# duxfrederic/lightcurver

Hardware: AMD Instinct MI355X
Metric: cutouts/sec (PSF-fit + joint forward-model iter), 32x32 & 64x64 stamps (higher is better)
Workload: dtype f32

## Files before the change

### include/lcmi.h

```cpp
#ifndef LCMI_H
#define LCMI_H

#include <stdint.h>

#ifdef __cplusplus
extern "C" {
#endif

#define LC_OK 0
#define LC_ERR_INVALID (-1)
#define LC_ERR_DEVICE (-2)
#define LC_ERR_UNSUPPORTED (-3)
#define LC_ERR_NONFINITE (-4)

typedef struct lc_ctx lc_ctx;
typedef struct lc_psf_batch lc_psf_batch;
typedef struct lc_joint lc_joint;

int lc_version(void);
int lc_ctx_create(int device, lc_ctx **out);
void lc_ctx_destroy(lc_ctx *ctx);
const char *lc_last_error(const lc_ctx *ctx);
int lc_ctx_synchronize(lc_ctx *ctx);
int lc_ctx_stream(lc_ctx *ctx, void **hip_stream, int *device);
// ... 37 lines not shown
                      int32_t *status , float *kernel_ms );

typedef struct {
  float n_sigma;
  int32_t clip;
} lc_stack_cfg;
int lc_align_stack_supported(int n);
int lc_align_stack(lc_ctx *ctx, int C, int E, int n, const float *cubes ,
                   const float *noisemap ,
                   const double *shift_yx , const double *angle_deg , const lc_stack_cfg *cfg,
                   float *aligned , float *stack ,
                   float *median , int32_t *n_rejected ,
                   float *kernel_ms );

typedef struct {
  float init_learning_rate;
  int32_t schedule_learning_rate;
  float decay_rate;
  int32_t transition_steps;
  float b1, b2, eps, eps_root;
} lc_adabelief_cfg;
void lc_adabelief_defaults(lc_adabelief_cfg *cfg);

int lc_psf_supported(int n, int ss);
int lc_psf_batch_create(lc_ctx *ctx, int F, int S_max, int n, int ss, const float *data,
                        const float *weight, lc_psf_batch **out);
void lc_psf_batch_destroy(lc_psf_batch *b);
int lc_psf_batch_set_moffat(lc_psf_batch *b, const float *moffat);
int lc_psf_batch_get_moffat(lc_psf_batch *b, float *moffat);
int lc_psf_batch_set_stars(lc_psf_batch *b, const float *stars);
int lc_psf_batch_get_stars(lc_psf_batch *b, float *stars);
int lc_psf_batch_set_grid(lc_psf_batch *b, const float *grid);
int lc_psf_batch_get_grid(lc_psf_batch *b, float *grid);
int lc_psf_batch_set_regularization(lc_psf_batch *b, const float *W, float lam_scales, float lam_hf);
int lc_psf_batch_propagate_noise(lc_psf_batch *b);
int lc_psf_batch_get_weights(lc_psf_batch *b, float *W);
int lc_psf_batch_eval(lc_psf_batch *b, float *loss, float *chi2, float *grad_moffat,
                      float *grad_stars, float *grad_grid, float *model);
int lc_psf_batch_fit_moffat(lc_psf_batch *b, int n_iter, float *final_loss );
int lc_psf_batch_run_adabelief(lc_psf_batch *b, int n_iter, const lc_adabelief_cfg *cfg);
int lc_psf_batch_iterations_done(lc_psf_batch *b);
int lc_psf_batch_split_fallbacks(lc_psf_batch *b, int *count);
int lc_psf_batch_get_loss_history(lc_psf_batch *b, float *history, int stride);
int lc_psf_batch_get_results(lc_psf_batch *b, float *narrow_psf, float *full_psf, float *residuals,
                             float *chi2);

int lc_psf_batch_set_moffat_q(lc_psf_batch *b, const float *q );
int lc_psf_batch_set_distortion(lc_psf_batch *frames, int S_stars, const float *coeffs ,
                                const float *xy );
int lc_psf_distortion_forward(lc_psf_batch *frames, lc_psf_batch *stars);
int lc_psf_distortion_backward(lc_psf_batch *frames, lc_psf_batch *stars);
int lc_psf_batch_get_ext_grad(lc_psf_batch *b, float *grad );
int lc_psf_batch_step_adabelief(lc_psf_batch *b, const lc_adabelief_cfg *cfg, int use_ext_grad, int export_grad);
int lc_psf_distortion_run(lc_psf_batch *frames, lc_psf_batch *stars, int n_iter, const lc_adabelief_cfg *cfg);
int lc_batched_lbfgs(int nb, int D, double *x, const double *lo, const double *hi, int maxiter,
                     int (*eval)(void *user, const double *X, double *F, double *G), void *user,
                     double *f_final , int *evaluations );

int lc_apply_distortion(lc_ctx *ctx, int N, int K, const float *narrow_psf, const float *coeffs,
                        const float *xy, float *out);

enum { LC_P_A = 0, LC_P_CX = 1, LC_P_CY = 2, LC_P_DX = 3, LC_P_DY = 4, LC_P_ALPHA = 5, LC_P_H = 6,
       LC_P_MEAN = 7, LC_P_COUNT = 8 };

typedef struct {
  float lam_scales, lam_hf;
// ... 72 lines not shown
```

### lightcurver_amd/_lib.py

```python
import ctypes as C
import os

import numpy as np

_HERE = os.path.dirname(os.path.abspath(__file__))
LIB_PATH = os.path.join(_HERE, 'liblcmi.so')

P_A, P_CX, P_CY, P_DX, P_DY, P_ALPHA, P_H, P_MEAN, P_COUNT = range(9)
PARAM_INDEX = {'a': P_A, 'c_x': P_CX, 'c_y': P_CY, 'dx': P_DX, 'dy': P_DY, 'alpha': P_ALPHA,
               'h': P_H, 'mean': P_MEAN}

fp = C.POINTER(C.c_float)
dp = C.POINTER(C.c_double)
ip = C.POINTER(C.c_int32)
vp = C.c_void_p
LBFGS_EVAL = C.CFUNCTYPE(C.c_int, C.c_void_p, dp, dp, dp)
ALLREDUCE_FN = C.CFUNCTYPE(C.c_int, C.c_void_p, C.c_void_p, C.c_int, C.c_void_p)
IPC_HANDLE_BYTES = 64
RCCL_ID_BYTES = 128


class AdabeliefCfg(C.Structure):
    _fields_ = [('init_learning_rate', C.c_float), ('schedule_learning_rate', C.c_int32),
                ('decay_rate', C.c_float), ('transition_steps', C.c_int32),
# ... 27 lines not shown
SIGNATURES = {
    'lc_version': (C.c_int, []),
    'lc_ctx_create': (C.c_int, [C.c_int, C.POINTER(vp)]),
    'lc_ctx_destroy': (None, [vp]),
    'lc_last_error': (C.c_char_p, [vp]),
    'lc_copy_bandwidth': (C.c_int, [vp, C.c_int64, C.c_int, C.POINTER(C.c_float)]),
    'lc_ctx_marker': (C.c_int, [vp, C.c_int]),
    'lc_prepare_stamps': (C.c_int, [vp, C.c_int, C.c_int, fp, fp, fp, fp, fp, C.POINTER(C.c_uint8), C.c_float, C.c_float,
                                    C.c_int, fp, fp, fp, C.POINTER(C.c_int32), C.POINTER(C.c_float)]),
    'lc_cosmics_supported': (C.c_int, [C.c_int]),
    'lc_detect_cosmics': (C.c_int, [vp, C.c_int, C.c_int, fp, fp, C.POINTER(C.c_uint8), C.POINTER(CosmicsCfg),
                                    C.POINTER(C.c_uint8), fp, ip, C.POINTER(C.c_float)]),
    'lc_segment_supported': (C.c_int, [C.c_int]),
    'lc_segment_stamps': (C.c_int, [vp, C.c_int, C.c_int, fp, fp, C.POINTER(SegmentCfg), C.POINTER(C.c_uint8), ip, ip, fp,
                                    ip, C.POINTER(C.c_float)]),
    'lc_align_stack_supported': (C.c_int, [C.c_int]),
    'lc_align_stack': (C.c_int, [vp, C.c_int, C.c_int, C.c_int, fp, fp, dp, dp, C.POINTER(StackCfg), fp, fp, fp, ip,
                                 C.POINTER(C.c_float)]),
    'lc_ctx_stream': (C.c_int, [vp, C.POINTER(C.c_void_p), C.POINTER(C.c_int)]),
    'lc_ctx_synchronize': (C.c_int, [vp]),
    'lc_timer_start': (C.c_int, [vp]),
    'lc_timer_stop': (C.c_int, [vp, fp]),
    'lc_device_info': (C.c_int, [vp, C.c_char_p, C.c_int, C.POINTER(C.c_int), C.POINTER(C.c_int64)]),
    'lc_adabelief_defaults': (None, [C.POINTER(AdabeliefCfg)]),
    'lc_psf_supported': (C.c_int, [C.c_int, C.c_int]),
    'lc_psf_batch_create': (C.c_int, [vp, C.c_int, C.c_int, C.c_int, C.c_int, fp, fp, C.POINTER(vp)]),
    'lc_psf_batch_destroy': (None, [vp]),
    'lc_psf_batch_set_moffat': (C.c_int, [vp, fp]),
    'lc_psf_batch_get_moffat': (C.c_int, [vp, fp]),
    'lc_psf_batch_set_stars': (C.c_int, [vp, fp]),
    'lc_psf_batch_get_stars': (C.c_int, [vp, fp]),
    'lc_psf_batch_set_grid': (C.c_int, [vp, fp]),
    'lc_psf_batch_get_grid': (C.c_int, [vp, fp]),
    'lc_psf_batch_set_regularization': (C.c_int, [vp, fp, C.c_float, C.c_float]),
    'lc_psf_batch_propagate_noise': (C.c_int, [vp]),
    'lc_psf_batch_get_weights': (C.c_int, [vp, fp]),
    'lc_psf_batch_eval': (C.c_int, [vp, fp, fp, fp, fp, fp, fp]),
    'lc_psf_batch_fit_moffat': (C.c_int, [vp, C.c_int, fp]),
    'lc_psf_batch_run_adabelief': (C.c_int, [vp, C.c_int, C.POINTER(AdabeliefCfg)]),
    'lc_psf_batch_iterations_done': (C.c_int, [vp]),
    'lc_psf_batch_split_fallbacks': (C.c_int, [vp, C.POINTER(C.c_int)]),
    'lc_psf_batch_get_loss_history': (C.c_int, [vp, fp, C.c_int]),
    'lc_psf_batch_get_results': (C.c_int, [vp, fp, fp, fp, fp]),
    'lc_psf_batch_set_moffat_q': (C.c_int, [vp, fp]),
    'lc_psf_batch_set_distortion': (C.c_int, [vp, C.c_int, fp, fp]),
    'lc_psf_distortion_forward': (C.c_int, [vp, vp]),
    'lc_psf_distortion_backward': (C.c_int, [vp, vp]),
    'lc_psf_batch_get_ext_grad': (C.c_int, [vp, fp]),
    'lc_psf_batch_step_adabelief': (C.c_int, [vp, C.POINTER(AdabeliefCfg), C.c_int, C.c_int]),
    'lc_psf_distortion_run': (C.c_int, [vp, vp, C.c_int, C.POINTER(AdabeliefCfg)]),
    'lc_batched_lbfgs': (C.c_int, [C.c_int, C.c_int, dp, dp, dp, C.c_int, LBFGS_EVAL, vp, dp, C.POINTER(C.c_int)]),
    'lc_apply_distortion': (C.c_int, [vp, C.c_int, C.c_int, fp, fp, fp, fp]),
    'lc_joint_supported': (C.c_int, [C.c_int, C.c_int]),
    'lc_joint_groups_background_supported': (C.c_int, [C.c_int, C.c_int]),
    'lc_joint_set_debug_global': (C.c_int, [C.c_int]),
    'lc_joint_create': (C.c_int, [vp, C.c_int, C.c_int, C.c_int, C.c_int, fp, fp, fp, C.POINTER(vp)]),
    'lc_joint_create_groups': (C.c_int, [vp, C.c_int, ip, C.c_int, C.c_int, C.c_int, fp, fp, fp, C.POINTER(vp)]),
    'lc_joint_create_groups_background': (C.c_int, [vp, C.c_int, ip, C.c_int, C.c_int, C.c_int, fp, fp, fp, C.POINTER(vp)]),
    'lc_joint_get_group_loss_history': (C.c_int, [vp, fp, C.c_int]),
    'lc_joint_destroy': (None, [vp]),
    'lc_joint_set_param': (C.c_int, [vp, C.c_int, fp, C.c_int]),
    'lc_joint_get_param': (C.c_int, [vp, C.c_int, fp, C.c_int]),
    'lc_joint_set_flux_reference': (C.c_int, [vp, fp, C.c_int]),
    'lc_joint_get_flux_reference': (C.c_int, [vp, fp, C.c_int]),
    'lc_joint_set_free': (C.c_int, [vp, ip]),
    'lc_joint_set_loss': (C.c_int, [vp, C.POINTER(JointLossCfg), fp]),
# ... 153 lines not shown
```

### lightcurver_amd/csrc/psf_batch.hip

```cpp
#include <cmath>
#include <cstring>

#include "lbfgs_host.h"
#include <thread>

#include "noise_host.h"
#include "starlet_norms.h"
#include <cstdlib>

#include "psf_kernels.h"
#include "psf_noise.h"
#include "psf_distort.h"
#include "psf_lbfgs.h"

using namespace lc;

struct lc_psf_batch {
  lc_ctx *ctx = nullptr;
  int F = 0, S = 0, n = 0, ss = 0, N = 0, J = 0;
  float *data = nullptr, *wgt = nullptr, *W = nullptr, *norms = nullptr, *Tm = nullptr;
  float *B = nullptr, *mB = nullptr, *sB = nullptr;
  float *stars = nullptr, *stars_m = nullptr, *stars_s = nullptr, *moffat = nullptr;
  float *hist = nullptr, *qscratch = nullptr;
  float *sched = nullptr;
// ... 536 lines not shown
}
int lc_psf_batch_get_moffat(lc_psf_batch *b, float *moffat) {
  if (!b || !moffat) return LC_ERR_INVALID;
  LC_ENTER(b->ctx);
  return d2h(b, moffat, b->moffat, (size_t)b->F * 4 * sizeof(float));
}
int lc_psf_batch_set_stars(lc_psf_batch *b, const float *stars) {
  if (!b || !stars) return LC_ERR_INVALID;
  LC_ENTER(b->ctx);
  return h2d(b, b->stars, stars, (size_t)b->F * b->S * 4 * sizeof(float));
}
int lc_psf_batch_get_stars(lc_psf_batch *b, float *stars) {
  if (!b || !stars) return LC_ERR_INVALID;
  LC_ENTER(b->ctx);
  return d2h(b, stars, b->stars, (size_t)b->F * b->S * 4 * sizeof(float));
}
int lc_psf_batch_set_grid(lc_psf_batch *b, const float *grid) {
  if (!b) return LC_ERR_INVALID;
  LC_ENTER(b->ctx);
  const size_t bytes = (size_t)b->F * b->N * b->N * sizeof(float);
  if (grid) return h2d(b, b->B, grid, bytes);
  LC_HIP(b->ctx, hipMemsetAsync(b->B, 0, bytes, b->ctx->stream));
  LC_HIP(b->ctx, hipMemsetAsync(b->mB, 0, bytes, b->ctx->stream));
  LC_HIP(b->ctx, hipMemsetAsync(b->sB, 0, bytes, b->ctx->stream));
  LC_HIP(b->ctx, hipMemsetAsync(b->stars_m, 0, (size_t)b->F * b->S * 4 * sizeof(float), b->ctx->stream));
  LC_HIP(b->ctx, hipMemsetAsync(b->stars_s, 0, (size_t)b->F * b->S * 4 * sizeof(float), b->ctx->stream));
  b->iters_done = 0;
  return LC_OK;
}
int lc_psf_batch_get_grid(lc_psf_batch *b, float *grid) {
  if (!b || !grid) return LC_ERR_INVALID;
  LC_ENTER(b->ctx);
  return d2h(b, grid, b->B, (size_t)b->F * b->N * b->N * sizeof(float));
}
int lc_psf_batch_set_regularization(lc_psf_batch *b, const float *W, float lam_scales, float lam_hf) {
  if (!b) return LC_ERR_INVALID;
  LC_ENTER(b->ctx);
  b->lam_sc = lam_scales;
  b->lam_hf = lam_hf;
  if (W) {
    int rc = h2d(b, b->W, W, (size_t)b->F * b->J * b->N * b->N * sizeof(float));
    if (rc) return rc;
    b->have_W = true;
  }
  return LC_OK;
}
namespace {
typedef void (*noise_fn)(int, int, const float *, const float *, const float *, float *);
noise_fn find_noise_kernel(int N, int ss) {
  if (N == 16 && ss == 1) return psf_noise_accumulate_kernel<16, 1>;
  if (N == 32 && ss == 2) return psf_noise_accumulate_kernel<32, 2>;
  if (N == 48 && ss == 2) return psf_noise_accumulate_kernel<48, 2>;
  if (N == 64 && ss == 2) return psf_noise_accumulate_kernel<64, 2>;
  if (N == 128 && ss == 2) return psf_noise_accumulate_kernel<128, 2>;
  return nullptr;
}
}

int lc_psf_batch_propagate_noise(lc_psf_batch *b) {
  if (!b) return LC_ERR_INVALID;
  LC_ENTER(b->ctx);
  const int F = b->F, S = b->S, N = b->N, n = b->n, ss = b->ss, J = b->J;
  const size_t NN = (size_t)N * N, nn = (size_t)n * n;
  if (!std::getenv("LCMI_NOISE_HOST")) {
    noise_fn fn = find_noise_kernel(N, ss);
    if (!fn) LC_FAIL(b->ctx, LC_ERR_UNSUPPORTED, "no noise-propagation kernel for this stamp size");
// ... 314 lines not shown
```

### lightcurver_amd/csrc/psf_kernels.h

```cpp
#pragma once
#include <utility>

#include "lc_common.h"
#include "starlet_device.h"

#ifndef LC_XPOLL_SLEEP
#define LC_XPOLL_SLEEP 2
#endif
namespace lc {
constexpr int kXFlagStride = 16;

#ifdef LC_STAMPS
__device__ long long g_stamps[128];
#define LC_STAMP(k)                                                      \
  do {                                                                   \
    if ((blockIdx.x == 0 || blockIdx.x == 8) && threadIdx.x == 0 && it == A.n_iter - 1)  \
      g_stamps[(k) + (blockIdx.x == 8 ? 64 : 0)] = clock64();            \
  } while (0)
#else
#define LC_STAMP(k) do {} while (0)
#endif


struct PsfArgs {
  int F, S, n_iter, t0, hist_stride, mode;
  const float *data, *wgt;
  const float *W;
  const float *norms;
  const float *Tm;
  float *B, *mB, *sB;
  float *stars, *stars_m, *stars_s;
  float *hist;
  float *qscratch;
  float *out_loss, *out_chi2, *out_gstars, *out_ggrid, *out_gT, *out_model;
  float lam_sc, lam_hf;
  lc_adabelief_cfg ab;
  float *xch;
  int *xflags, *xabort;
  int launch_seq, heal, force_abort_it;
  const float *bkB, *bkmB, *bksB, *bkstars, *bkstars_m, *bkstars_s;
// ... 27 lines not shown
               : "memory");
}
__device__ __forceinline__ void load_sc1_x4(const float *p, lc_v4f &a) {
  asm volatile("global_load_dwordx4 %0, %1, off sc1\n\ts_waitcnt vmcnt(0)" : "=&v"(a) : "v"(p) : "memory");
}
__device__ __forceinline__ float load_sc1_f(const float *p) {
  float v;
  asm volatile("global_load_dword %0, %1, off sc1\n\ts_waitcnt vmcnt(0)" : "=&v"(v) : "v"(p) : "memory");
  return v;
}


template <int N_, int SS_, int PX_, int SG_, bool WC_ = false, int JB_ = 8>
struct PsfCfg {
  static constexpr int N = N_, SS = SS_, PX = PX_, SG = SG_;
  static constexpr bool WC = WC_;
  static constexpr int n = N / SS;
  static constexpr int NTHR = N * N / PX;
  static constexpr int NW = (NTHR + kWave - 1) / kWave;
  static constexpr int NT = ntaps(SS);
  static constexpr int J = ilog2(N);
  static constexpr int LR = 8;
  static constexpr int LC = (JB_ * (N_ / SS_) / 4 >= 64) ? 4 : 2;
  static constexpr int LA = LC;
  static constexpr int TS = N + 1;
  static constexpr int RS = n + 1;
  static constexpr int OFF_T = 0;
  static constexpr int SZ_T = WC_ ? N * (N + 2 * (N / 4 + 10) + 1) : N * TS;
  static constexpr int OFF_R = OFF_T + SZ_T;
  static constexpr int SZ_R2 = SG * n * TS;
  static constexpr int VS = WC_ ? n + 3 : RS, VO = WC_ ? 1 : 0;
  static constexpr int SZ_V = SG * N * VS;
  static constexpr int JB = JB_;
  static constexpr int AP = N / 4 + 10;
  static constexpr int TSA = N + 2 * AP + 1;
  static constexpr int APR = AP / SS + 2;
  static constexpr int JBP = JB + 1;
  static constexpr int WSZ = JB * TSA + (n + 2 * APR) * JBP;
  static constexpr int SZ_VR = (SZ_V > StarletLds<N>::FLOATS) ? SZ_V : StarletLds<N>::FLOATS;
  static constexpr int OFF_WSC = OFF_R + SZ_VR;
  static constexpr int SZ_R = WC ? (SZ_VR + NW * WSZ) : ((2 * SZ_R2 > SZ_V) ? 2 * SZ_R2 : SZ_V);
  static constexpr int OFF_RES = OFF_R + SZ_R;
  static constexpr int SZ_RES = WC ? 0 : SG * n * n;
  static constexpr int OFF_TAPS = OFF_RES + SZ_RES;
  static constexpr int NTP = NT + 3;
  static constexpr int SZ_TAPS = (16 * 4 * NTP + 1) / 2 * 2 + 16 * 2 * NT * 2;
  static constexpr int OFF_TAPP = OFF_TAPS + (16 * 4 * NTP + 1) / 2 * 2;
  static constexpr int OFF_RED = OFF_TAPS + SZ_TAPS;
  static constexpr int IPS = n * n / LC;
  static constexpr int IPS_PAD = (IPS + kWave - 1) / kWave * kWave;
  static constexpr int SLOTS = IPS_PAD / kWave;
  static constexpr int SZ_REDX = 16 * NW;
  static constexpr int SZ_RED = (WC ? 16 * (n / JB) * 5 : SG * SLOTS * 5) + SZ_REDX + NW + 8;
  static constexpr int OFF_REDX = OFF_RED + (WC ? 16 * (n / JB) * 5 : SG * SLOTS * 5);
  static constexpr int OFF_REDW = OFF_REDX + SZ_REDX;
  static constexpr int OFF_STAR = OFF_RED + SZ_RED;
  static constexpr int MAXS = 16;
  static constexpr int SZ_STAR = MAXS * 20 + 16;
  static constexpr int LDS_FLOATS = OFF_STAR + SZ_STAR;
  static_assert(WC || StarletLds<N>::FLOATS <= SZ_T + SZ_R + SZ_RES, "starlet ping-pong buffers must fit over T + R + RES");
  static_assert(PX % SS == 0 && N % PX == 0 && n % LR == 0 && n % LC == 0 && n % LA == 0 && n % JB == 0, "tiling");
  static_assert(LDS_FLOATS * 4 <= 163840, "LDS");
  static_assert(OFF_TAPP % 2 == 0, "tap pairs are read as 64-bit words");
  static_assert(NTHR <= 1024 && NTHR % kWave == 0, "threads");
  static_assert(!WC_ || PX_ <= 8, "the WC layout keeps the pixel state in registers");
};


template <int SS, int NT>
__device__ inline void tap_entry(float delta, int k, float &tap, float &dtap, int &bq) {
  const int o = (int)nearbyintf(delta);
  const int base = o - kRg - (SS - 1);
  int q = base / SS;
  if (q * SS > base) --q;
  bq = q;
  const int m = q * SS + k;
  const float inv_s2 = 1.0f / (kSigmaG * kSigmaG);
  const float nrm = 0.3989422804014327f / kSigmaG;
  float a = 0.f, d = 0.f;
#pragma unroll
  for (int dv = 0; dv < SS; ++dv) {
    const int t = m + dv;
    if (t >= o - kRg && t <= o + kRg) {
      const float x = (float)t - delta;
      const float p = nrm * expf(-0.5f * x * x * inv_s2);
      a += p;
      d += p * x * inv_s2;
    }
  }
  tap = a;
  dtap = d;
}

template <class C, bool SPLIT = false>
__global__ __launch_bounds__(C::NTHR) void psf_fit_kernel(PsfArgs A) {
  constexpr int N = C::N, SS = C::SS, PX = C::PX, SG = C::SG, n = C::n, NT = C::NT, J = C::J;
  constexpr int NTHR = C::NTHR, TS = C::TS, RS = C::RS, LR = C::LR, LC = C::LC, LA = C::LA;
  extern __shared__ __align__(16) float lds[];
  float *T = lds + C::OFF_T;
  float *R2t = lds + C::OFF_R;
  float *R2xt = R2t + C::SZ_R2;
  float *V = lds + C::OFF_R;
  float *RES = lds + C::OFF_RES;
  float *TAPS = lds + C::OFF_TAPS + 1;
  constexpr int NTP = C::NTP;
  lc_v2f *TAPP = (lc_v2f *)(lds + C::OFF_TAPP);
  float *REDX = lds + C::OFF_REDX;
  float *RED = lds + C::OFF_RED;
  float *REDW = lds + C::OFF_REDW;
  float *SCAL = REDW + C::NW;
  float *SP = lds + C::OFF_STAR;
  float *SGR = SP + C::MAXS * 4;
  float *SM = SGR + C::MAXS * 5;
  float *SV = SM + C::MAXS * 4;
  int *BQ = (int *)(SV + C::MAXS * 4);

  int f = blockIdx.x, role = 0;
  if constexpr (SPLIT) {
    f = ((int)blockIdx.x >> 4) * 8 + ((int)blockIdx.x & 7);
    role = ((int)blockIdx.x >> 3) & 1;
    if (f >= A.F) return;
  }
  const bool conv_role = !SPLIT || role == 0, starlet_role = !SPLIT || role == 1;
  const int my_xcc = SPLIT ? (int)(__builtin_amdgcn_s_getreg(20 | (3 << 11)) & 15u) : 0;
  int same_xcd = 0;
  const int tid0 = threadIdx.x;
// ... 122 lines not shown
    float tpix[PX];
    if (conv_role) {
    if (C::WC && STATE_REGS) {
#pragma unroll
      for (int p = 0; p < PX; ++p) {
        tpix[p] = Bp[p] + Tp[p];
        T[pu * C::TSA + C::AP + pv + p] = tpix[p];
      }
    } else if (STATE_REGS) {
#pragma unroll
      for (int p = 0; p < PX; ++p) T[pu * TS + pv + p] = Bp[p] + Tp[p];
    } else {
      const float4 *bp = (const float4 *)(Bg + gpix);
      const float4 *tp = (const float4 *)(A.Tm + gpix);
#pragma unroll
      for (int q = 0; q < PX / 4; ++q) {
        const float4 b = bp[q], t = tp[q];
        T[pu * TS + pv + 4 * q + 0] = b.x + t.x;
        T[pu * TS + pv + 4 * q + 1] = b.y + t.y;
        T[pu * TS + pv + 4 * q + 2] = b.z + t.z;
        T[pu * TS + pv + 4 * q + 3] = b.w + t.w;
      }
    }
    if (tid < S * 5) SGR[tid] = 0.f;

    for (int g0 = 0; g0 < S; g0 += SG) {
      __syncthreads();
      LC_STAMP(1 + 5 * (g0 / SG));
      if constexpr (C::WC) {
        constexpr int JB = C::JB, NBLK = n / JB;
        float *wsc = lds + C::OFF_WSC + wid * C::WSZ;
        constexpr int TSA = C::TSA, AP = C::AP, APR = C::APR;
        float *R2w = wsc + AP, *RESw = wsc + JB * TSA + APR * C::JBP;
        int kdone = 0;
        for (int task = wid; task < SG * NBLK; task += C::NW, ++kdone) {
          progress_prio(kdone);
          const int sl = task / NBLK, blk = task % NBLK, s = g0 + sl;
          if (s >= S) continue;
          const int jd0 = blk * JB;
          const float *tx = TAPS + (s * 4 + 0) * NTP, *ty = tx + 2 * NTP, *dty = tx + 3 * NTP;
          const int bqx = BQ[s * 2 + 0], bqy = BQ[s * 2 + 1];
          const float amp = SP[s * 4 + 0], sky = SP[s * 4 + 3];
          constexpr int NI3 = (JB * (n / LC) + 63) / 64;
          float dpre[NI3][LC], wpre[NI3][LC];
#pragma unroll
          for (int i3 = 0; i3 < NI3; ++i3) {
            const int item = lane + 64 * i3;
            const bool ok = item < JB * (n / LC);
            const int jl = item % JB, a0 = (item / JB) * LC;
#pragma unroll
            for (int j = 0; j < LC; ++j) {
              const size_t pix = ok ? ((size_t)s * n * n + (size_t)(a0 + j) * n + jd0 + jl) : 0;
              const float dv = dataf[pix], wv = wgtf[pix];
              dpre[i3][j] = ok ? dv : 0.f;
              wpre[i3][j] = ok ? wv : 0.f;
            }
          }
          LC_STAMP(10);
          {
            const int ws = SS * (jd0 - bqx) - (NT - 1);
            if constexpr (SS == 2) {
              constexpr int NP = (NT + 1) / 2, WL2 = (JB - 1) + NP;
              lc_v2f tr2[NP];
#pragma unroll
              for (int h = 0; h < NP; ++h) tr2[h] = (lc_v2f){tx[NT - 1 - 2 * h], tx[NT - 2 - 2 * h]};
              for (int u = lane; u < N; u += 64) {
                lc_v2f win2[WL2];
                const float *trow = T + u * TSA + AP + ws;
#pragma unroll
                for (int i = 0; i < WL2; ++i) win2[i] = (lc_v2f){trow[2 * i], trow[2 * i + 1]};
                lc_v2f acc[JB];
#pragma unroll
                for (int j = 0; j < JB; ++j) acc[j] = (lc_v2f){0.f, 0.f};
#pragma unroll
                for (int h = 0; h < NP; ++h) {
#pragma unroll
                  for (int j = 0; j < JB; ++j) acc[j] = pk_fma(tr2[h], win2[j + h], acc[j]);
                }
#pragma unroll
                for (int j = 0; j < JB; ++j) R2w[j * TSA + u] = acc[j].x + acc[j].y;
              }
            } else {
              constexpr int WL = SS * (JB - 1) + NT;
              float tk[NT];
#pragma unroll
              for (int k = 0; k < NT; ++k) tk[k] = tx[k];
              for (int u = lane; u < N; u += 64) {
                float win[WL];
                const float *trow = T + u * TSA + AP + ws;
#pragma unroll
                for (int i = 0; i < WL; ++i) win[i] = trow[i];
#pragma unroll
                for (int j = 0; j < JB; ++j) {
                  float acc = 0.f;
#pragma unroll
                  for (int k = 0; k < NT; ++k) acc = fmaf(tk[k], win[SS * j - k + NT - 1], acc);
                  R2w[j * TSA + u] = acc;
                }
              }
            }
          }
          wave_lds_sync();
          LC_STAMP(11);
          float chi = 0.f, ga = 0.f, gy = 0.f, gs = 0.f;
          {
            constexpr int WL = SS * (LC - 1) + NT;
            lc_v2f tyd[NT];
#pragma unroll
            for (int k = 0; k < NT; ++k) tyd[k] = TAPP[(s * 2 + 1) * NT + k];
#pragma unroll
// ... 14 lines not shown
                for (int k = 0; k < NT; ++k) {
#pragma unroll
                  for (int j = 0; j < LC; ++j) fvys[j] = pk_fma(tyd[k], pk_bcast(win[SS * j - k + NT - 1]), fvys[j]);
                  if constexpr (LC == 4) asm volatile("" : "+v"(fvys[0]), "+v"(fvys[1]), "+v"(fvys[2]), "+v"(fvys[3]));
                  else asm volatile("" : "+v"(fvys[0]), "+v"(fvys[1]));
                }
#pragma unroll
                for (int j = 0; j < LC; ++j) {
                  const float fv = fvys[j].x, fy = fvys[j].y;
                  const float model = fmaf(amp, fv, sky);
                  const float res = model - dpre[i3][j];
                  const float rw = wpre[i3][j] * res;
                  chi = fmaf(rw, res, chi);
                  ga = fmaf(rw, fv, ga);
                  lgy = fmaf(rw, fy, lgy);
                  gs += rw;
                  RESw[(a0 + j) * C::JBP + jl] = rw;
                  if (A.out_model) A.out_model[(size_t)f * S * n * n + (size_t)s * n * n + (size_t)(a0 + j) * n + jd0 + jl] = model;
                }
                gy += lgy * amp * SS;
              }
            }
          }
          wave_sum4(chi, ga, gy, gs);
          if (lane == 0) {
            float *r = RED + (s * NBLK + blk) * 5;
            r[0] = chi;
            r[1] = ga;
            r[3] = gy;
            r[4] = gs;
          }
          wave_lds_sync();
          LC_STAMP(12);
          {
            constexpr int WI = (SS * LA - 1 + NT - 1) / SS + 1;
            constexpr int NI4 = (JB * (n / LA) + 63) / 64;
            if constexpr (SS == 2) {
              constexpr int NP = (NT + 1) / 2;
              lc_v2f py[NP];
#pragma unroll
              for (int q = 0; q < NP; ++q) py[q] = (lc_v2f){ty[2 * q], ty[2 * q - 1]};
#pragma unroll
              for (int i4 = 0; i4 < NI4; ++i4) {
                const int item = lane + 64 * i4;
                if (item < JB * (n / LA)) {
                  const int jl = item % JB, a0 = (item / JB) * LA;
                  lc_v2f out2[LA];
#pragma unroll
                  for (int h = 0; h < LA; ++h) out2[h] = (lc_v2f){0.f, 0.f};
                  const float *rcol = RESw + (bqy + a0) * C::JBP + jl;
#pragma unroll
                  for (int i = 0; i < WI; ++i) {
                    const lc_v2f rv = pk_bcast(rcol[i * C::JBP]);
#pragma unroll
                    for (int h = 0; h < LA; ++h)
                      if (i - h >= 0 && i - h < NP) out2[h] = pk_fma(py[i - h], rv, out2[h]);
                  }
                  float *vrow = V + (sl * N + SS * a0) * C::VS + C::VO + jd0 + jl;
#pragma unroll
                  for (int h = 0; h < LA; ++h) {
                    vrow[(2 * h) * C::VS] = out2[h].x;
                    vrow[(2 * h + 1) * C::VS] = out2[h].y;
                  }
                  if (jd0 + jl == 0) {
#pragma unroll
                    for (int r = 0; r < SS * LA; ++r) V[(sl * N + SS * a0 + r) * C::VS] = 0.f;
// ... 20 lines not shown
#pragma unroll
                  for (int i = 0; i < WI; ++i) {
                    const float rv = rcol[i * C::JBP];
#pragma unroll
                    for (int k = 0; k < NT; ++k) {
                      const int rel = SS * i - k;
                      if (rel >= 0 && rel < SS * LA) out[rel] = fmaf(tk[k], rv, out[rel]);
                    }
                  }
#pragma unroll
                  for (int r = 0; r < SS * LA; ++r) V[(sl * N + SS * a0 + r) * C::VS + C::VO + jd0 + jl] = out[r];
                  if (jd0 + jl == 0) {
#pragma unroll
                    for (int r = 0; r < SS * LA; ++r) V[(sl * N + SS * a0 + r) * C::VS] = 0.f;
                  }
                  if (jd0 + jl == n - 1) {
#pragma unroll
                    for (int r = 0; r < SS * LA; ++r) V[(sl * N + SS * a0 + r) * C::VS + n + 1] = 0.f;
                  }
                }
              }
            }
          }
          wave_lds_sync();
          LC_STAMP(13);
        }
        __builtin_amdgcn_s_setprio(0);
        LC_STAMP(14);
#ifdef LC_STAMPS
        if (blockIdx.x == 0 && lane == 0 && it == A.n_iter - 1) g_stamps[20 + wid] = clock64();
#endif
        __syncthreads();
        LC_STAMP(15);
        if (tid < SG * 5) {
          const int sl = tid / 5, q = tid % 5;
          if (g0 + sl < S && q != 2) {
            float acc = 0.f;
            for (int k = 0; k < NBLK; ++k) acc += RED[((g0 + sl) * NBLK + k) * 5 + q];
            SGR[(g0 + sl) * 5 + q] = acc;
          }
        }
      } else {
      constexpr int NIT3 = (SG * C::IPS_PAD + NTHR - 1) / NTHR;
      float dpre[NIT3][LC], wpre[NIT3][LC];
#pragma unroll
      for (int i3 = 0; i3 < NIT3; ++i3) {
        const int item0 = wid * 64 + i3 * NTHR, item = item0 + lane;
        const int sl = item0 / C::IPS_PAD, within = item % C::IPS_PAD, s = g0 + sl;
        const bool ok = (item0 < SG * C::IPS_PAD) && (s < S) && (within < C::IPS);
        const int jd = within % n, a0 = (within / n) * LC;
#pragma unroll
        for (int j = 0; j < LC; ++j) {
          const size_t pix = ok ? ((size_t)s * n * n + (size_t)(a0 + j) * n + jd) : 0;
          const float dv = dataf[pix], wv = wgtf[pix];
          dpre[i3][j] = ok ? dv : 0.f;
          wpre[i3][j] = ok ? wv : 0.f;
        }
      }
      {
        constexpr int WL = SS * (LR - 1) + NT;
        constexpr int NSTRIP = n / LR;
        for (int item = tid; item < SG * N * NSTRIP; item += NTHR) {
          const int u = item % N, strip = (item / N) % NSTRIP, sl = item / (N * NSTRIP);
          if (g0 + sl >= S) continue;
          const float *tx = TAPS + ((g0 + sl) * 4 + 0) * NTP;
          const int bq = BQ[(g0 + sl) * 2 + 0];
          const int a0 = strip * LR;
          const int ws = SS * (a0 - bq) - (NT - 1);
// ... 109 lines not shown
          const int jd = item % n, strip = (item / n) % NSTRIP, sl = item / (n * NSTRIP);
          if (g0 + sl >= S) continue;
          const float *ty = TAPS + ((g0 + sl) * 4 + 2) * NTP;
          const int bq = BQ[(g0 + sl) * 2 + 1];
          const int a0 = strip * LA;
          float tk[NT];
#pragma unroll
          for (int k = 0; k < NT; ++k) tk[k] = ty[k];
          float out[SS * LA];
#pragma unroll
          for (int r = 0; r < SS * LA; ++r) out[r] = 0.f;
#pragma unroll
          for (int i = 0; i < WI; ++i) {
            const int id = i + bq + a0;
            const int ci = min(max(id, 0), n - 1);
            float rv = RES[(sl * n + ci) * n + jd];
            rv = (id >= 0 && id < n) ? rv : 0.f;
#pragma unroll
            for (int k = 0; k < NT; ++k) {
              const int rel = SS * i - k;
              if (rel >= 0 && rel < SS * LA) out[rel] = fmaf(tk[k], rv, out[rel]);
            }
          }
#pragma unroll
          for (int r = 0; r < SS * LA; ++r) V[(sl * N + SS * a0 + r) * RS + jd] = out[r];
        }
      }
      __syncthreads();
      LC_STAMP(4 + 5 * (g0 / SG));
      }
      LC_STAMP(16);
      if constexpr (C::WC) {
        constexpr int WJ = (PX - 1 + NT - 1) / SS + 1;
        for (int sl = 0; sl < SG; ++sl) {
          const int s = g0 + sl;
          if (s >= S) break;
          progress_prio((4 * sl) / SG);
          const float *tx = TAPS + (s * 4 + 0) * NTP, *dtx = tx + NTP;
          const int bq = BQ[s * 2 + 0];
          const float amp = SP[s * 4 + 0];
          lc_v2f txd[NT];
#pragma unroll
          for (int k = 0; k < NT; ++k) txd[k] = TAPP[(s * 2 + 0) * NT + k];
          lc_v2f accp[PX];
#pragma unroll
          for (int p = 0; p < PX; ++p) accp[p] = (lc_v2f){0.f, 0.f};
          const float *vrow = V + (sl * N + pu) * C::VS + 1;
          const int jd0 = bq + pv / SS;
          float vwin[WJ];
#pragma unroll
          for (int i = 0; i < WJ; ++i) vwin[i] = vrow[min(max(jd0 + i, -1), n)];
#pragma unroll
          for (int i = 0; i < WJ; ++i) {
            const lc_v2f vv = pk_bcast(vwin[i]);
#pragma unroll
            for (int k = 0; k < NT; ++k) {
              const int rel = SS * i - k;
              if (rel >= 0 && rel < PX) accp[rel] = pk_fma(txd[k], vv, accp[rel]);
            }
          }
          float gxs = 0.f;
#pragma unroll
          for (int p = 0; p < PX; ++p) {
            gB[p] = fmaf(amp, accp[p].x, gB[p]);
            gxs = fmaf(accp[p].y, tpix[p], gxs);
          }
          gxs = wave_sum(gxs);
          if (lane == 0) REDX[s * C::NW + wid] = gxs;
        }
        __builtin_amdgcn_s_setprio(0);
      } else {
        constexpr int WJ = (PX - 1 + NT - 1) / SS + 1;
        for (int sl = 0; sl < SG; ++sl) {
          const int s = g0 + sl;
          if (s >= S) break;
          const float *tx = TAPS + (s * 4 + 0) * NTP, *dtx = tx + NTP;
          const int bq = BQ[s * 2 + 0];
          const float amp = SP[s * 4 + 0];
          float acc[PX], gxs = 0.f;
#pragma unroll
          for (int p = 0; p < PX; ++p) acc[p] = 0.f;
#pragma unroll
          for (int i = 0; i < WJ; ++i) {
            const int jd = i + bq + pv / SS;
            const int ci = min(max(jd, 0), n - 1);
            float vv = V[(sl * N + pu) * RS + ci];
            vv = (jd >= 0 && jd < n) ? vv : 0.f;
            float dsum = 0.f;
#pragma unroll
            for (int k = 0; k < NT; ++k) {
              const int rel = SS * i - k;
              if (rel >= 0 && rel < PX) {
                acc[rel] = fmaf(tx[k], vv, acc[rel]);
                dsum = fmaf(dtx[k], T[pu * TS + pv + rel], dsum);
              }
            }
            gxs = fmaf(vv, dsum, gxs);
          }
#pragma unroll
          for (int p = 0; p < PX; ++p) gB[p] = fmaf(amp, acc[p], gB[p]);
          gxs = wave_sum(gxs);
// ... 224 lines not shown
```

### lightcurver_amd/psf_batch.py

```python
import ctypes as C

import numpy as np

from . import _lib
from ._lib import f32, ptr


class PsfBatch:

    def __init__(self, data, weight, ss, ctx=None):
        data = f32(data)
        weight = f32(weight)
        if data.ndim != 4 or data.shape != weight.shape or data.shape[2] != data.shape[3]:
            raise ValueError('data and weight must be (F, S, n, n)')
        self.ctx = ctx or _lib.default_context()
        self._l = _lib.lib()
        self.F, self.S, self.n, _ = data.shape
        self.ss = int(ss)
        self.N = self.n * self.ss
        self.J = int(np.log2(self.N))
        if not self._l.lc_psf_supported(self.n, self.ss):
            raise _lib.LcError(f'no PSF kernel for stamp size n={self.n}, subsampling {self.ss}')
        h = C.c_void_p()
        self.ctx.check(self._l.lc_psf_batch_create(self.ctx.h, self.F, self.S, self.n, self.ss, ptr(data),
# ... 29 lines not shown

    def distortion_run(self, stars, n_iter, **cfg):
        c = _lib.adabelief_cfg(**cfg)
        self._chk(self._l.lc_psf_distortion_run(self.h, stars.h, int(n_iter), C.byref(c)), 'distortion_run')

    def get_ext_grad(self):
        g = np.empty((self.F, self.N, self.N), np.float32)
        self._chk(self._l.lc_psf_batch_get_ext_grad(self.h, ptr(g)), 'get_ext_grad')
        return g

    def step_adabelief(self, use_ext_grad=False, export_grad=False, **cfg):
        c = _lib.adabelief_cfg(**cfg)
        self._chk(self._l.lc_psf_batch_step_adabelief(self.h, C.byref(c), int(bool(use_ext_grad)), int(bool(export_grad))),
                  'step_adabelief')

    def set_stars(self, stars):
        s = f32(stars).reshape(self.F, self.S, 4)
        self._chk(self._l.lc_psf_batch_set_stars(self.h, ptr(s)), 'set_stars')

    def get_stars(self):
        s = np.empty((self.F, self.S, 4), np.float32)
        self._chk(self._l.lc_psf_batch_get_stars(self.h, ptr(s)), 'get_stars')
        return s

    def set_grid(self, grid=None):
        g = None if grid is None else f32(grid).reshape(self.F, self.N * self.N)
        self._chk(self._l.lc_psf_batch_set_grid(self.h, ptr(g)), 'set_grid')

    def get_grid(self):
        g = np.empty((self.F, self.N, self.N), np.float32)
        self._chk(self._l.lc_psf_batch_get_grid(self.h, ptr(g)), 'get_grid')
        return g

    def set_regularization(self, W=None, lam_scales=1.0, lam_hf=1.0):
        w = None if W is None else f32(W).reshape(self.F, self.J, self.N, self.N)
        self._chk(self._l.lc_psf_batch_set_regularization(self.h, ptr(w), float(lam_scales), float(lam_hf)),
                  'set_regularization')

    def propagate_noise(self):
        self._chk(self._l.lc_psf_batch_propagate_noise(self.h), 'propagate_noise')

    def get_weights(self):
        w = np.empty((self.F, self.J, self.N, self.N), np.float32)
        self._chk(self._l.lc_psf_batch_get_weights(self.h, ptr(w)), 'get_weights')
        return w

    def evaluate(self, model=False):
        F, S, n, N = self.F, self.S, self.n, self.N
        out = dict(loss=np.empty(F, np.float32), chi2=np.empty(F, np.float32),
                   grad_moffat=np.empty((F, 4), np.float32), grad_stars=np.empty((F, S, 4), np.float32),
                   grad_grid=np.empty((F, N, N), np.float32))
        mod = np.empty((F, S, n, n), np.float32) if model else None
        self._chk(self._l.lc_psf_batch_eval(self.h, ptr(out['loss']), ptr(out['chi2']), ptr(out['grad_moffat']),
                                            ptr(out['grad_stars']), ptr(out['grad_grid']), ptr(mod)), 'eval')
        if model:
            out['model'] = mod
        return out

    def fit_moffat(self, n_iter):
        fl = np.empty(self.F, np.float32)
        self._chk(self._l.lc_psf_batch_fit_moffat(self.h, int(n_iter), ptr(fl)), 'fit_moffat')
        return fl

    def run_adabelief(self, n_iter, **cfg):
        c = _lib.adabelief_cfg(**cfg)
        self._chk(self._l.lc_psf_batch_run_adabelief(self.h, int(n_iter), C.byref(c)), 'run_adabelief')
# ... 39 lines not shown
```

Baseline: 57.86 million.

## Software-pipeline per-star parameter loads and batch wave sums in PSF fit kernel

Adds an LC_PIPE bitmask, on by default, that enables prefetching of the next task's per-star parameters (BQ, SP, taps) one iteration ahead in the WC convolution loop. It also prefetches the next star's taps and V window in the phase-5 gradient loop. Four stars' x0 sums are combined in one wave_sum4 reduction, and the per-star sum reduction moves to the last wave. These changes aim to hide global/LDS load latency and cut cross-lane reduction overhead, at the cost of extra registers, which may lower occupancy. A get_moments API for reading optimizer moments is added as well.

Result: slower. 55.85 million (-3.5%).

```diff
diff --git a/include/lcmi.h b/include/lcmi.h
--- a/include/lcmi.h
+++ b/include/lcmi.h
@@ -93,6 +93,7 @@
 int lc_psf_batch_get_stars(lc_psf_batch *b, float *stars);
 int lc_psf_batch_set_grid(lc_psf_batch *b, const float *grid);
 int lc_psf_batch_get_grid(lc_psf_batch *b, float *grid);
+int lc_psf_batch_get_moments(lc_psf_batch *b, float *grid_m, float *grid_s, float *stars_m, float *stars_s);
 int lc_psf_batch_set_regularization(lc_psf_batch *b, const float *W, float lam_scales, float lam_hf);
 int lc_psf_batch_propagate_noise(lc_psf_batch *b);
 int lc_psf_batch_get_weights(lc_psf_batch *b, float *W);
diff --git a/lightcurver_amd/_lib.py b/lightcurver_amd/_lib.py
--- a/lightcurver_amd/_lib.py
+++ b/lightcurver_amd/_lib.py
@@ -83,6 +83,7 @@
     'lc_psf_batch_get_stars': (C.c_int, [vp, fp]),
     'lc_psf_batch_set_grid': (C.c_int, [vp, fp]),
     'lc_psf_batch_get_grid': (C.c_int, [vp, fp]),
+    'lc_psf_batch_get_moments': (C.c_int, [vp, fp, fp, fp, fp]),
     'lc_psf_batch_set_regularization': (C.c_int, [vp, fp, C.c_float, C.c_float]),
     'lc_psf_batch_propagate_noise': (C.c_int, [vp]),
     'lc_psf_batch_get_weights': (C.c_int, [vp, fp]),
diff --git a/lightcurver_amd/csrc/psf_batch.hip b/lightcurver_amd/csrc/psf_batch.hip
--- a/lightcurver_amd/csrc/psf_batch.hip
+++ b/lightcurver_amd/csrc/psf_batch.hip
@@ -592,6 +592,17 @@
   if (!b || !grid) return LC_ERR_INVALID;
   LC_ENTER(b->ctx);
   return d2h(b, grid, b->B, (size_t)b->F * b->N * b->N * sizeof(float));
+}
+int lc_psf_batch_get_moments(lc_psf_batch *b, float *grid_m, float *grid_s, float *stars_m, float *stars_s) {
+  if (!b) return LC_ERR_INVALID;
+  LC_ENTER(b->ctx);
+  const size_t gb = (size_t)b->F * b->N * b->N * sizeof(float), sb = (size_t)b->F * b->S * 4 * sizeof(float);
+  int rc;
+  if (grid_m && (rc = d2h(b, grid_m, b->mB, gb))) return rc;
+  if (grid_s && (rc = d2h(b, grid_s, b->sB, gb))) return rc;
+  if (stars_m && (rc = d2h(b, stars_m, b->stars_m, sb))) return rc;
+  if (stars_s && (rc = d2h(b, stars_s, b->stars_s, sb))) return rc;
+  return LC_OK;
 }
 int lc_psf_batch_set_regularization(lc_psf_batch *b, const float *W, float lam_scales, float lam_hf) {
   if (!b) return LC_ERR_INVALID;
diff --git a/lightcurver_amd/csrc/psf_kernels.h b/lightcurver_amd/csrc/psf_kernels.h
--- a/lightcurver_amd/csrc/psf_kernels.h
+++ b/lightcurver_amd/csrc/psf_kernels.h
@@ -6,6 +6,9 @@
 
 #ifndef LC_XPOLL_SLEEP
 #define LC_XPOLL_SLEEP 2
+#endif
+#ifndef LC_PIPE
+#define LC_PIPE 15
 #endif
 namespace lc {
 constexpr int kXFlagStride = 16;
@@ -99,6 +102,7 @@
   static constexpr int VS = WC_ ? n + 3 : RS, VO = WC_ ? 1 : 0;
   static constexpr int SZ_V = SG * N * VS;
   static constexpr int JB = JB_;
+  static constexpr bool PIPE = WC_ && PX_ == 8;
   static constexpr int AP = N / 4 + 10;
   static constexpr int TSA = N + 2 * AP + 1;
   static constexpr int APR = AP / SS + 2;
@@ -159,6 +163,27 @@
   dtap = d;
 }
 
+template <class C>
+struct WcTaskPre {
+  static constexpr int NPR = (C::SS == 2) ? (C::NT + 1) / 2 : 1;
+  lc_v2f tr2[NPR];
+  int bqx, bqy;
+  float amp, sky;
+};
+template <class C>
+__device__ __forceinline__ void wc_task_request(int s, const float *TAPS, const int *BQ, const float *SP, WcTaskPre<C> &q) {
+  constexpr int NT = C::NT;
+  q.bqx = BQ[s * 2 + 0];
+  q.bqy = BQ[s * 2 + 1];
+  q.amp = SP[s * 4 + 0];
+  q.sky = SP[s * 4 + 3];
+  if constexpr (C::SS == 2) {
+    const float *tx = TAPS + (s * 4 + 0) * C::NTP;
+#pragma unroll
+    for (int h = 0; h < WcTaskPre<C>::NPR; ++h) q.tr2[h] = (lc_v2f){tx[NT - 1 - 2 * h], tx[NT - 2 - 2 * h]};
+  }
+}
+
 template <class C, bool SPLIT = false>
 __global__ __launch_bounds__(C::NTHR) void psf_fit_kernel(PsfArgs A) {
   constexpr int N = C::N, SS = C::SS, PX = C::PX, SG = C::SG, n = C::n, NT = C::NT, J = C::J;
@@ -347,6 +372,15 @@
         float *wsc = lds + C::OFF_WSC + wid * C::WSZ;
         constexpr int TSA = C::TSA, AP = C::AP, APR = C::APR;
         float *R2w = wsc + AP, *RESw = wsc + JB * TSA + APR * C::JBP;
+        constexpr int NI3 = (JB * (n / LC) + 63) / 64;
+        constexpr bool TASK_AHEAD = C::PIPE && (LC_PIPE & 4) != 0;
+        using TaskPre = WcTaskPre<C>;
+        TaskPre ahead;
+        auto task_ahead = [&](int task) {
+          const int sl = task / NBLK;
+          wc_task_request<C>((task < SG * NBLK && g0 + sl < S) ? g0 + sl : 0, TAPS, BQ, SP, ahead);
+        };
+        if constexpr (TASK_AHEAD) task_ahead(wid);
         int kdone = 0;
         for (int task = wid; task < SG * NBLK; task += C::NW, ++kdone) {
           progress_prio(kdone);
@@ -354,9 +388,11 @@
           if (s >= S) continue;
           const int jd0 = blk * JB;
           const float *tx = TAPS + (s * 4 + 0) * NTP, *ty = tx + 2 * NTP, *dty = tx + 3 * NTP;
-          const int bqx = BQ[s * 2 + 0], bqy = BQ[s * 2 + 1];
-          const float amp = SP[s * 4 + 0], sky = SP[s * 4 + 3];
-          constexpr int NI3 = (JB * (n / LC) + 63) / 64;
+          TaskPre tp;
+          if constexpr (TASK_AHEAD) tp = ahead;
+          else wc_task_request<C>(s, TAPS, BQ, SP, tp);
+          const int bqx = tp.bqx, bqy = tp.bqy;
+          const float amp = tp.amp, sky = tp.sky;
           float dpre[NI3][LC], wpre[NI3][LC];
 #pragma unroll
           for (int i3 = 0; i3 < NI3; ++i3) {
@@ -375,10 +411,7 @@
           {
             const int ws = SS * (jd0 - bqx) - (NT - 1);
             if constexpr (SS == 2) {
-              constexpr int NP = (NT + 1) / 2, WL2 = (JB - 1) + NP;
-              lc_v2f tr2[NP];
-#pragma unroll
-              for (int h = 0; h < NP; ++h) tr2[h] = (lc_v2f){tx[NT - 1 - 2 * h], tx[NT - 2 - 2 * h]};
+              constexpr int NP = TaskPre::NPR, WL2 = (JB - 1) + NP;
               for (int u = lane; u < N; u += 64) {
                 lc_v2f win2[WL2];
                 const float *trow = T + u * TSA + AP + ws;
@@ -390,7 +423,7 @@
 #pragma unroll
                 for (int h = 0; h < NP; ++h) {
 #pragma unroll
-                  for (int j = 0; j < JB; ++j) acc[j] = pk_fma(tr2[h], win2[j + h], acc[j]);
+                  for (int j = 0; j < JB; ++j) acc[j] = pk_fma(tp.tr2[h], win2[j + h], acc[j]);
                 }
 #pragma unroll
                 for (int j = 0; j < JB; ++j) R2w[j * TSA + u] = acc[j].x + acc[j].y;
@@ -471,6 +504,10 @@
           }
           wave_lds_sync();
           LC_STAMP(12);
+          if constexpr (TASK_AHEAD) {
+            task_ahead(task + C::NW);
+            __builtin_amdgcn_sched_barrier(0);
+          }
           {
             constexpr int WI = (SS * LA - 1 + NT - 1) / SS + 1;
             constexpr int NI4 = (JB * (n / LA) + 63) / 64;
@@ -557,8 +594,11 @@
 #endif
         __syncthreads();
         LC_STAMP(15);
-        if (tid < SG * 5) {
-          const int sl = tid / 5, q = tid % 5;
+        constexpr bool SUMS_LAST = C::PIPE && (LC_PIPE & 8) != 0;
+        static_assert(SG * 5 <= 64, "the per-star sums are one wave's");
+        const int ts = SUMS_LAST ? tid - (NTHR - 64) : tid;
+        if (ts < SG * 5 && (!SUMS_LAST || ts >= 0)) {
+          const int sl = ts / 5, q = ts % 5;
           if (g0 + sl < S && q != 2) {
             float acc = 0.f;
             for (int k = 0; k < NBLK; ++k) acc += RED[((g0 + sl) * NBLK + k) * 5 + q];
@@ -734,41 +774,114 @@
       LC_STAMP(16);
       if constexpr (C::WC) {
         constexpr int WJ = (PX - 1 + NT - 1) / SS + 1;
-        for (int sl = 0; sl < SG; ++sl) {
-          const int s = g0 + sl;
-          if (s >= S) break;
-          progress_prio((4 * sl) / SG);
-          const float *tx = TAPS + (s * 4 + 0) * NTP, *dtx = tx + NTP;
-          const int bq = BQ[s * 2 + 0];
-          const float amp = SP[s * 4 + 0];
-          lc_v2f txd[NT];
-#pragma unroll
-          for (int k = 0; k < NT; ++k) txd[k] = TAPP[(s * 2 + 0) * NT + k];
-          lc_v2f accp[PX];
-#pragma unroll
-          for (int p = 0; p < PX; ++p) accp[p] = (lc_v2f){0.f, 0.f};
-          const float *vrow = V + (sl * N + pu) * C::VS + 1;
-          const int jd0 = bq + pv / SS;
-          float vwin[WJ];
-#pragma unroll
-          for (int i = 0; i < WJ; ++i) vwin[i] = vrow[min(max(jd0 + i, -1), n)];
-#pragma unroll
-          for (int i = 0; i < WJ; ++i) {
-            const lc_v2f vv = pk_bcast(vwin[i]);
-#pragma unroll
-            for (int k = 0; k < NT; ++k) {
-              const int rel = SS * i - k;
-              if (rel >= 0 && rel < PX) accp[rel] = pk_fma(txd[k], vv, accp[rel]);
-            }
-          }
-          float gxs = 0.f;
-#pragma unroll
-          for (int p = 0; p < PX; ++p) {
-            gB[p] = fmaf(amp, accp[p].x, gB[p]);
-            gxs = fmaf(accp[p].y, tpix[p], gxs);
-          }
-          gxs = wave_sum(gxs);
-          if (lane == 0) REDX[s * C::NW + wid] = gxs;
+        if constexpr (C::PIPE) {
+          constexpr bool P5_AHEAD = C::PIPE && (LC_PIPE & 1) != 0, P5_SUMS = C::PIPE && (LC_PIPE & 2) != 0;
+          constexpr int QS = P5_SUMS ? 4 : 1;
+          static_assert(SG % QS == 0, "wave_sum4 takes the stars' x0 sums four at a time");
+          struct P5Star {
+            lc_v2f txd[NT];
+            float vwin[WJ], amp;
+          };
+          auto p5_request = [&](int sl, P5Star &q) {
+            const int slc = min(sl, min(S - 1 - g0, SG - 1)), s = g0 + slc;
+            const int bq = BQ[s * 2 + 0];
+            q.amp = SP[s * 4 + 0];
+#pragma unroll
+            for (int k = 0; k < NT; ++k) q.txd[k] = TAPP[(s * 2 + 0) * NT + k];
+            const float *vrow = V + (slc * N + pu) * C::VS + 1;
+            const int jd0 = bq + pv / SS;
+#pragma unroll
+            for (int i = 0; i < WJ; ++i) q.vwin[i] = vrow[min(max(jd0 + i, -1), n)];
+          };
+          P5Star cur, nxt;
+          if constexpr (P5_AHEAD) p5_request(0, cur);
+#pragma unroll 1
+          for (int q0 = 0; q0 < SG; q0 += QS) {
+            if (g0 + q0 >= S) break;
+            float gx[QS];
+#pragma unroll
+            for (int j = 0; j < QS; ++j) gx[j] = 0.f;
+#pragma unroll
+            for (int j = 0; j < QS; ++j) {
+              const int sl = q0 + j, s = g0 + sl;
+              if (s >= S) break;
+              progress_prio((4 * sl) / SG);
+              if constexpr (P5_AHEAD) {
+                p5_request(sl + 1, nxt);
+                __builtin_amdgcn_sched_barrier(0);
+              } else {
+                p5_request(sl, cur);
+              }
+              lc_v2f accp[PX];
+#pragma unroll
+              for (int p = 0; p < PX; ++p) accp[p] = (lc_v2f){0.f, 0.f};
+#pragma unroll
+              for (int i = 0; i < WJ; ++i) {
+                const lc_v2f vv = pk_bcast(cur.vwin[i]);
+#pragma unroll
+                for (int k = 0; k < NT; ++k) {
+                  const int rel = SS * i - k;
+                  if (rel >= 0 && rel < PX) accp[rel] = pk_fma(cur.txd[k], vv, accp[rel]);
+                }
+              }
+              float gxs = 0.f;
+#pragma unroll
+              for (int p = 0; p < PX; ++p) {
+                gB[p] = fmaf(cur.amp, accp[p].x, gB[p]);
+                gxs = fmaf(accp[p].y, tpix[p], gxs);
+              }
+              gx[j] = gxs;
+              if constexpr (P5_AHEAD) cur = nxt;
+            }
+            if constexpr (P5_SUMS) {
+              wave_sum4(gx[0], gx[1], gx[2], gx[3]);
+              if (lane == 0) {
+#pragma unroll
+                for (int j = 0; j < QS; ++j)
+                  if (g0 + q0 + j < S) REDX[(g0 + q0 + j) * C::NW + wid] = gx[j];
+              }
+            } else {
+              const float gxw = wave_sum(gx[0]);
+              if (lane == 0) REDX[(g0 + q0) * C::NW + wid] = gxw;
+            }
+          }
+        } else {
+          for (int sl = 0; sl < SG; ++sl) {
+            const int s = g0 + sl;
+            if (s >= S) break;
+            progress_prio((4 * sl) / SG);
+            const float *tx = TAPS + (s * 4 + 0) * NTP, *dtx = tx + NTP;
+            const int bq = BQ[s * 2 + 0];
+            const float amp = SP[s * 4 + 0];
+            lc_v2f txd[NT];
+#pragma unroll
+            for (int k = 0; k < NT; ++k) txd[k] = TAPP[(s * 2 + 0) * NT + k];
+            lc_v2f accp[PX];
+#pragma unroll
+            for (int p = 0; p < PX; ++p) accp[p] = (lc_v2f){0.f, 0.f};
+            const float *vrow = V + (sl * N + pu) * C::VS + 1;
+            const int jd0 = bq + pv / SS;
+            float vwin[WJ];
+#pragma unroll
+            for (int i = 0; i < WJ; ++i) vwin[i] = vrow[min(max(jd0 + i, -1), n)];
+#pragma unroll
+            for (int i = 0; i < WJ; ++i) {
+              const lc_v2f vv = pk_bcast(vwin[i]);
+#pragma unroll
+              for (int k = 0; k < NT; ++k) {
+                const int rel = SS * i - k;
+                if (rel >= 0 && rel < PX) accp[rel] = pk_fma(txd[k], vv, accp[rel]);
+              }
+            }
+            float gxs = 0.f;
+#pragma unroll
+            for (int p = 0; p < PX; ++p) {
+              gB[p] = fmaf(amp, accp[p].x, gB[p]);
+              gxs = fmaf(accp[p].y, tpix[p], gxs);
+            }
+            gxs = wave_sum(gxs);
+            if (lane == 0) REDX[s * C::NW + wid] = gxs;
+          }
         }
         __builtin_amdgcn_s_setprio(0);
       } else {
diff --git a/lightcurver_amd/psf_batch.py b/lightcurver_amd/psf_batch.py
--- a/lightcurver_amd/psf_batch.py
+++ b/lightcurver_amd/psf_batch.py
@@ -85,6 +85,13 @@
         self._chk(self._l.lc_psf_batch_get_grid(self.h, ptr(g)), 'get_grid')
         return g
 
+    def get_moments(self):
+        out = dict(grid_m=np.empty((self.F, self.N, self.N), np.float32), grid_s=np.empty((self.F, self.N, self.N), np.float32),
+                   stars_m=np.empty((self.F, self.S, 4), np.float32), stars_s=np.empty((self.F, self.S, 4), np.float32))
+        self._chk(self._l.lc_psf_batch_get_moments(self.h, ptr(out['grid_m']), ptr(out['grid_s']), ptr(out['stars_m']),
+                                                   ptr(out['stars_s'])), 'get_moments')
+        return out
+
     def set_regularization(self, W=None, lam_scales=1.0, lam_hf=1.0):
         w = None if W is None else f32(W).reshape(self.F, self.J, self.N, self.N)
         self._chk(self._l.lc_psf_batch_set_regularization(self.h, ptr(w), float(lam_scales), float(lam_hf)),
```
